# williamyang98/SDRPlusPlus-DAB-Radio-Plugin

Measured on AMD Instinct MI355X. Metric: DAB Mode-I frames/sec (OFDM+Viterbi), higher is better.
Workload: dtype f32

## Files before the change

sdrplusplus-dab-radio-plugin_amd/csrc/dabgpu_ctx.hpp:

```cpp
#pragma once
#include "../../include/dabgpu.h"

#include <hip/hip_runtime.h>

#include <chrono>
#include <map>
#include <memory>
#include <vector>

#include "dab_tables.hpp"
#include "kernels.hpp"
#include "iq_load.hpp"

namespace dabapi {

struct DeviceCode {
    dab::PunctureProfile prof;
    uint16_t *d_mother_pos = nullptr;
    uint8_t *d_prbs = nullptr;
    int32_t *d_punct_idx = nullptr;
    int32_t *d_fused_desc = nullptr, *d_fused_tiles = nullptr;
    dabk::LaneTables lane_tables() const { return dabk::LaneTables{d_punct_idx, d_fused_desc, d_fused_tiles}; }
    dabk::CodeTables tables(bool descramble) const {
        const bool chunked = d_mother_pos && prof.nsteps >= 102 && (prof.nsteps - 6) % 96 == 0;
// ... 41 lines not shown
    std::map<uint64_t, dabapi::DeviceCode *> code_by_descriptor;
    void *d_stage[9] = {nullptr, nullptr, nullptr, nullptr, nullptr, nullptr, nullptr, nullptr, nullptr};
    size_t stage_bytes[9] = {0, 0, 0, 0, 0, 0, 0, 0, 0};
    bool timing = false;
    dabapi::Timer timers[4];
    int ofdm_parts_override = 0;
    const unsigned long long *d_keep = nullptr;
    std::vector<void *> keep_tables;
    void *d_acq_scratch = nullptr;
    size_t acq_scratch_bytes = 0;
    void *d_lane_scratch = nullptr;
    size_t lane_scratch_bytes = 0;
    int lane_mode = -1;
    bool lane_unfused = false;
    bool test_one_domain = false;
    int test_fail_in = 0;
    int wave_slots = 3072;
    std::vector<dabgpu_bit_range> keep_ranges;
    dabk::StreamState *d_states = nullptr;
    int n_states = 0;
    hipEvent_t ev_states = nullptr;
    bool ev_states_pending = false;
    float thr_null_start = 0.35f;
    float signal_beta = 0.95f;
    bool loop_dd = false;
    float dd_gate = 2.5f;
    int keep_symbols = 75;
    struct SubHistory {
        int start_address, length;
        size_t bytes;
        int8_t *ring[2];
        int cur;
        bool live;
    };
    std::vector<SubHistory> sub_history;
    void *h_bounce = nullptr;
    size_t h_bounce_bytes = 0;
    unsigned long long signal_seq = 0;
    dabapi::Arena arena;
    dabapi::Pipeline *pipe = nullptr;
    int iq_format = 0;
};

namespace dabapi {

struct DeviceGuard {
    int prev = -1;
    bool switched = false;
    explicit DeviceGuard(const dabgpu_ctx *ctx) {
        if (ctx && hipGetDevice(&prev) == hipSuccess && prev != ctx->device) switched = hipSetDevice(ctx->device) == hipSuccess;
    }
    ~DeviceGuard() {
        if (switched) (void)hipSetDevice(prev);
    }
    DeviceGuard(const DeviceGuard &) = delete;
    DeviceGuard &operator=(const DeviceGuard &) = delete;
};

#define HIP_TRY(expr)                               \
    do {                                            \
        hipError_t e_ = (expr);                     \
        if (e_ != hipSuccess) return DABGPU_ERR_HIP; \
    } while (0)

struct ScopedTimer {
    dabgpu_ctx *ctx;
    int which;
    hipStream_t s;
    ScopedTimer(dabgpu_ctx *c, int w, hipStream_t st) : ctx(c), which(w), s(st) {
        if (ctx->timing) {
            Timer &t = ctx->timers[which];
            const int i = int(t.recorded % TIMER_RING);
            if (!t.start[i]) { (void)hipEventCreate(&t.start[i]); (void)hipEventCreate(&t.stop[i]); }
            t.has_mid[i] = false;
            (void)hipEventRecord(t.start[i], s);
        }
    }
    hipEvent_t *mids() {
        if (!ctx->timing) return nullptr;
        Timer &t = ctx->timers[which];
        const int i = int(t.recorded % TIMER_RING);
        for (hipEvent_t &e : t.mid[i])
            if (!e && hipEventCreate(&e) != hipSuccess) return nullptr;
        t.has_mid[i] = true;
        return t.mid[i];
    }
    ~ScopedTimer() {
        if (ctx->timing) {
            Timer &t = ctx->timers[which];
            (void)hipEventRecord(t.stop[int(t.recorded % TIMER_RING)], s);
            t.recorded++;
        }
    }
};

constexpr long SIGNAL_SPIN_US = 200;
inline int wait_for_signal(hipStream_t s, volatile unsigned long long *flag_host, unsigned long long *flag_dev, unsigned long long seq,
                           bool already_signalled = false, bool results_coherent = true) {
    if (!results_coherent) return hipStreamSynchronize(s) == hipSuccess ? DABGPU_OK : DABGPU_ERR_HIP;
    if (!already_signalled && dabk::launch_signal(flag_dev, seq, s) != hipSuccess) return DABGPU_ERR_HIP;
    const auto give_up = std::chrono::steady_clock::now() + std::chrono::microseconds(SIGNAL_SPIN_US);
    for (;;) {
        for (int i = 0; i < 64; i++) {
            if (*flag_host == seq) {
                __atomic_thread_fence(__ATOMIC_ACQUIRE);
                return DABGPU_OK;
            }
#if defined(__x86_64__) || defined(__i386__)
            __builtin_ia32_pause();
#endif
        }
        if (std::chrono::steady_clock::now() >= give_up) break;
    }
    return hipStreamSynchronize(s) == hipSuccess ? DABGPU_OK : DABGPU_ERR_HIP;
}

inline bool injected_failure(dabgpu_ctx *ctx) {
    return ctx->test_fail_in > 0 && --ctx->test_fail_in == 0;
}

inline hipStream_t pick_stream(dabgpu_ctx *ctx, void *stream) {
    return stream ? reinterpret_cast<hipStream_t>(stream) : ctx->stream;
}

int stage(dabgpu_ctx *ctx, int slot, size_t bytes, void **out);
int get_code(dabgpu_ctx *ctx, dab::PunctureProfile &&prof, DeviceCode **out);
void free_device_code(DeviceCode &dc);
void *device_alias_of_pinned(const void *host);
bool known_coherent_host(const void *host, size_t bytes);
int ensure_bounce(dabgpu_ctx *ctx, size_t bytes);
int note_state_use(dabgpu_ctx *ctx, hipStream_t s);
int wait_state_use(dabgpu_ctx *ctx);
void stats_of(const dabk::StreamState &st, dabgpu_stats *out);
void arena_destroy(dabgpu_ctx *ctx);
void pipeline_destroy(dabgpu_ctx *ctx);

inline bool subchannels_disjoint(const dabgpu_subchannel *sc, int n) {
    char used[864] = {};
    for (int i = 0; i < n; i++) {
        if (sc[i].start_address < 0 || sc[i].length <= 0 || sc[i].start_address + sc[i].length > 864) return false;
        for (int cu = sc[i].start_address; cu < sc[i].start_address + sc[i].length; cu++) {
            if (used[cu]) return false;
            used[cu] = 1;
        }
    }
    return true;
}

constexpr int LANE_MIN_CODEWORDS = 24576;

}
```

sdrplusplus-dab-radio-plugin_amd/csrc/dabgpu_decode_api.hip:

```cpp
#include "dabgpu_ctx.hpp"

#include <algorithm>
#include <cstring>

using namespace dab;
using namespace dabapi;

namespace {

bool use_lane(dabgpu_ctx *ctx, int nsteps, int n_codewords, hipStream_t s, dabk::LaneScratch *sc, int *rc, bool force = false) {
    *rc = DABGPU_OK;
    if (!dabk::lane_supported(nsteps)) return false;
    if (!force && (ctx->lane_mode == 0 || (ctx->lane_mode < 0 && n_codewords < LANE_MIN_CODEWORDS))) return false;
    const size_t need = dabk::lane_scratch_bytes(nsteps, n_codewords);
    if (ctx->lane_scratch_bytes < need) {
        if (hipStreamSynchronize(s) != hipSuccess) { *rc = DABGPU_ERR_HIP; return false; }
        if (ctx->d_lane_scratch) (void)hipFree(ctx->d_lane_scratch);
        ctx->d_lane_scratch = nullptr;
        ctx->lane_scratch_bytes = 0;
        if (hipMalloc(&ctx->d_lane_scratch, need) != hipSuccess) {
            ctx->d_lane_scratch = nullptr;
            if (ctx->lane_mode > 0 || force) *rc = DABGPU_ERR_NOMEM;
            return false;
        }
// ... 176 lines not shown
    if (nframes == 0) return DABGPU_OK;
    const size_t nb_soft = (nframes - 1) * soft_stride + NB_FRAME_BITS;
    const size_t nb_hist = size_t(n_streams) * 15 * sc->length * CU_BITS;
    const size_t nb_out = nframes * NB_CIFS * nbytes;
    void *d_soft, *d_hi = nullptr, *d_ho = nullptr, *d_out;
    int rc;
    if ((rc = stage(ctx, 1, nb_soft, &d_soft))) return rc;
    if ((rc = stage(ctx, 3, nb_out, &d_out))) return rc;
    if (history_in && (rc = stage(ctx, 4, nb_hist, &d_hi))) return rc;
    if (history_out && (rc = stage(ctx, 5, nb_hist, &d_ho))) return rc;
    hipStream_t s = ctx->stream;
    HIP_TRY(hipMemcpyAsync(d_soft, soft, nb_soft, hipMemcpyHostToDevice, s));
    if (history_in) HIP_TRY(hipMemcpyAsync(d_hi, history_in, nb_hist, hipMemcpyHostToDevice, s));
    rc = dabgpu_msc_decode_dev(ctx, sc, static_cast<const int8_t *>(d_soft), soft_stride, n_streams,
                               frames_per_stream, static_cast<const int8_t *>(d_hi), static_cast<int8_t *>(d_ho),
                               static_cast<uint8_t *>(d_out), s);
    if (rc) return rc;
    HIP_TRY(hipMemcpyAsync(out, d_out, nb_out, hipMemcpyDeviceToHost, s));
    if (history_out) HIP_TRY(hipMemcpyAsync(history_out, d_ho, nb_hist, hipMemcpyDeviceToHost, s));
    HIP_TRY(hipStreamSynchronize(s));
    return DABGPU_OK;
}

static int decode_grouped(dabgpu_ctx *ctx, uint8_t *d_fib, uint8_t *d_crc_ok, const dabgpu_subchannel *sc, int n_subchannels,
                          const int8_t *d_soft, size_t soft_stride, int n_streams, int frames_per_stream,
                          const int8_t *const *d_history_in, int8_t *const *d_history_out, uint8_t *const *d_out,
                          void *stream) {
    const int n_items = n_subchannels + (d_fib ? 1 : 0);
    if (n_items < 2 || ctx->lane_mode == 0 || ctx->lane_unfused || !d_soft || n_streams <= 0 || frames_per_stream <= 0 ||
        soft_stride < size_t(NB_FRAME_BITS))
        return 1;
    const long total_cw = long(n_items) * n_streams * frames_per_stream * NB_CIFS;
    if (ctx->lane_mode < 0 && total_cw < LANE_MIN_CODEWORDS) return 1;
    std::vector<dabk::LaneGroupItem> items;
    if (d_fib) {
        dabk::LaneGroupItem it{};
        it.code = ctx->fic.tables(true);
        it.tables = ctx->fic.lane_tables();
        it.args.soft = d_soft;
        it.args.soft_stride = soft_stride;
        it.args.n_streams = n_streams;
        it.args.frames_per_stream = frames_per_stream;
        it.args.out = d_fib;
        it.is_fic = true;
        it.crc_ok = d_crc_ok;
        if (((reinterpret_cast<uintptr_t>(d_soft) | soft_stride) & 15) || (reinterpret_cast<uintptr_t>(d_fib) & 3)) return 1;
        items.push_back(it);
    }
    for (int i = 0; i < n_subchannels; i++) {
        DeviceCode *dc = nullptr;
        const int rc = lookup_code(ctx, &sc[i], &dc);
        if (rc) return rc;
        dabk::LaneGroupItem it{};
        it.code = dc->tables(true);
        it.tables = dc->lane_tables();
        it.args.soft = d_soft;
        it.args.soft_stride = soft_stride;
        it.args.n_streams = n_streams;
        it.args.frames_per_stream = frames_per_stream;
        it.args.start_bit = sc[i].start_address * CU_BITS;
        it.args.nbits = sc[i].length * CU_BITS;
        it.args.hist_in = d_history_in ? d_history_in[i] : nullptr;
        it.args.hist_out = d_history_out ? d_history_out[i] : nullptr;
        it.args.out = d_out[i];
        if (it.args.hist_in && it.args.hist_in == it.args.hist_out) return DABGPU_ERR_ARG;
        if (!dabk::lane_supported(dc->prof.nsteps) || !dabk::lane_group_fusable(it.args)) return 1;
        items.push_back(it);
    }
    hipStream_t s = pick_stream(ctx, stream);
    const size_t need = dabk::lane_group_scratch_bytes(items.data(), n_items);
    if (ctx->lane_scratch_bytes < need) {
        HIP_TRY(hipStreamSynchronize(s));
        if (ctx->d_lane_scratch) (void)hipFree(ctx->d_lane_scratch);
        ctx->d_lane_scratch = nullptr;
        ctx->lane_scratch_bytes = 0;
        if (hipMalloc(&ctx->d_lane_scratch, need) != hipSuccess) {
            ctx->d_lane_scratch = nullptr;
            return 1;
        }
        ctx->lane_scratch_bytes = need;
    }
    ScopedTimer tm(ctx, 2, s);
    dabk::LaneScratch lsc{ctx->d_lane_scratch, ctx->lane_scratch_bytes};
    HIP_TRY(dabk::launch_lane_group(items.data(), n_items, lsc, s, tm.mids()));
    for (const dabk::LaneGroupItem &it : items)
        if (!it.is_fic) HIP_TRY(dabk::launch_msc_history(it.args, s));
    return 0;
}

static int decode_subchannels(dabgpu_ctx *ctx, const dabgpu_subchannel *sc, int n_subchannels, const int8_t *d_soft,
                              size_t soft_stride, int n_streams, int frames_per_stream, const int8_t *const *d_history_in,
                              int8_t *const *d_history_out, uint8_t *const *d_out, void *stream, uint8_t *d_fib = nullptr,
                              uint8_t *d_crc_ok = nullptr) {
    const long cw_each = long(n_streams) * frames_per_stream * NB_CIFS;
    bool group = n_subchannels >= 1 && n_subchannels + (d_fib ? 1 : 0) >= 2 && ctx->lane_mode <= 0 &&
                 (ctx->lane_mode == 0 || cw_each < LANE_MIN_CODEWORDS) && d_soft && n_streams > 0 && frames_per_stream > 0;
    std::vector<dabk::WaveGroupItem> items;
    for (int i = 0; group && i < n_subchannels; i++) {
        DeviceCode *dc = nullptr;
        const int rc = lookup_code(ctx, &sc[i], &dc);
        if (rc) return rc;
        if (!dabk::wave_group_supported(dc->prof.nsteps)) { group = false; break; }
        dabk::WaveGroupItem it{};
        it.code = dc->tables(true);
        it.args.soft = d_soft;
        it.args.soft_stride = soft_stride;
        it.args.n_streams = n_streams;
        it.args.frames_per_stream = frames_per_stream;
        it.args.start_bit = sc[i].start_address * CU_BITS;
        it.args.nbits = sc[i].length * CU_BITS;
        it.args.hist_in = d_history_in ? d_history_in[i] : nullptr;
        it.args.hist_out = d_history_out ? d_history_out[i] : nullptr;
        it.args.out = d_out[i];
        if (it.args.hist_in && it.args.hist_in == it.args.hist_out) return DABGPU_ERR_ARG;
        items.push_back(it);
    }
    if (group && n_subchannels == 1 && !dabk::wave_group_one_round(std::max(items[0].code.nsteps, ctx->fic.prof.nsteps), 2 * cw_each))
        group = false;
    if (group) {
        hipStream_t s = pick_stream(ctx, stream);
        ScopedTimer tm(ctx, 2, s);
        dabk::WaveFicItem fic{ctx->fic.tables(true), d_soft, soft_stride, n_streams * frames_per_stream, d_fib, d_crc_ok};
        HIP_TRY(dabk::launch_msc_decode_group(items.data(), int(items.size()), s, d_fib ? &fic : nullptr));
        return DABGPU_OK;
    }
    if (d_fib) {
        const int rc = dabgpu_fic_decode_dev(ctx, d_soft, soft_stride, n_streams * frames_per_stream, d_fib, d_crc_ok, stream);
        if (rc) return rc;
    }
    for (int i = 0; i < n_subchannels; i++) {
        const int rc = dabgpu_msc_decode_dev(ctx, &sc[i], d_soft, soft_stride, n_streams, frames_per_stream,
                                             d_history_in ? d_history_in[i] : nullptr,
                                             d_history_out ? d_history_out[i] : nullptr, d_out[i], stream);
        if (rc) return rc;
    }
    return DABGPU_OK;
}

int dabgpu_msc_decode_multi_dev(dabgpu_ctx *ctx, const dabgpu_subchannel *sc, int n_subchannels,
                                const int8_t *d_soft, size_t soft_stride, int n_streams, int frames_per_stream,
                                const int8_t *const *d_history_in, int8_t *const *d_history_out,
                                uint8_t *const *d_out, void *stream) {
    if (!ctx || !sc || !d_out || n_subchannels < 0) return DABGPU_ERR_ARG;
    DeviceGuard guard(ctx);
    std::vector<char> used(864, 0);
    for (int i = 0; i < n_subchannels; i++) {
        DeviceCode *dc = nullptr;
        const int rc = lookup_code(ctx, &sc[i], &dc);
        if (rc) return rc;
        if (!d_out[i]) return DABGPU_ERR_ARG;
        for (int cu = sc[i].start_address; cu < sc[i].start_address + sc[i].length; cu++) {
            if (used[cu]) return DABGPU_ERR_ARG;
            used[cu] = 1;
        }
    }
    {
        const int g = decode_grouped(ctx, nullptr, nullptr, sc, n_subchannels, d_soft, soft_stride, n_streams,
                                     frames_per_stream, d_history_in, d_history_out, d_out, stream);
        if (g <= 0) return g;
    }
    return decode_subchannels(ctx, sc, n_subchannels, d_soft, soft_stride, n_streams, frames_per_stream, d_history_in,
                              d_history_out, d_out, stream);
}

int dabgpu_decode_frames_dev(dabgpu_ctx *ctx, const int8_t *d_soft, size_t soft_stride, int n_streams,
                             int frames_per_stream, uint8_t *d_fib, uint8_t *d_crc_ok, const dabgpu_subchannel *sc,
                             int n_subchannels, const int8_t *const *d_history_in, int8_t *const *d_history_out,
// ... 452 lines not shown
```

sdrplusplus-dab-radio-plugin_amd/csrc/kernels.hpp:

```cpp
#pragma once
#include <hip/hip_runtime.h>

#include <vector>
#include <cstddef>
#include <cstdint>

namespace dabk {

struct OfdmTables {
    const float2 *twiddle;
    const uint16_t *bin_of_n;
    const uint16_t *n_of_vj;
};

struct StreamState {
    float fine_freq_offset;
    float coarse_freq_offset;
    float signal_average;
    float last_fine_error;
    int32_t total_frames_read;
    int32_t total_frames_desync;
    int32_t tracking;
    int32_t last_time_offset;
    double next_frame_start;
// ... 168 lines not shown
                              int max_out, int64_t advance, int only_lost, hipStream_t s);

struct SuperframeStatus {
    int32_t firecode_ok;
    int32_t rs_corrected;
    int32_t rs_uncorrectable;
    int32_t num_aus;
    int32_t au_crc_mask;
    int32_t au_start[8];
    int32_t reserved[3];
};
hipError_t launch_dabplus_superframes(const uint8_t *in, size_t in_stride, int n_superframes, int s, uint8_t *out,
                                      SuperframeStatus *status, hipStream_t stream, unsigned long long *done_flag = nullptr,
                                      unsigned long long done_seq = 0);

struct CodeTables {
    const uint16_t *mother_pos;
    int n_punct;
    int nsteps;
    const uint8_t *prbs_bytes;
    const uint16_t *chunk_first = nullptr;
};
__host__ __device__ inline int code_chunk_table_offset(int n_punct) { return (n_punct + 7) & ~7; }

hipError_t launch_fic_decode(const CodeTables &c, const int8_t *soft, size_t soft_stride, int n_frames,
                             uint8_t *fib, uint8_t *crc_ok, hipStream_t s);
hipError_t launch_viterbi_plain(const CodeTables &c, const int8_t *punct, int n_codewords, uint8_t *out,
                                hipStream_t s);
struct MscArgs {
    const int8_t *soft;
    size_t soft_stride;
    int n_streams;
    int frames_per_stream;
    int start_bit;
    int nbits;
    const int8_t *hist_in;
    int8_t *hist_out;
    uint8_t *out;
};
hipError_t launch_msc_decode(const CodeTables &c, const MscArgs &a, hipStream_t s);
struct WaveGroupItem {
    CodeTables code;
    MscArgs args;
};
struct WaveFicItem {
    CodeTables code;
    const int8_t *soft;
    size_t soft_stride;
    int n_frames;
    uint8_t *fib, *crc_ok;
};
bool wave_group_supported(int nsteps);
bool wave_group_one_round(int max_nsteps, long n_waves);
hipError_t launch_msc_decode_group(const WaveGroupItem *items, int n, hipStream_t s, const WaveFicItem *fic = nullptr);

struct LaneScratch {
    void *base;
    size_t bytes;
    bool unfused = false;
};
size_t lane_scratch_bytes(int nsteps, int n_codewords);
bool lane_supported(int nsteps);
struct LaneTables {
    const int32_t *punct_idx;
    const int32_t *fused_desc;
    const int32_t *fused_tiles;
};
void build_lane_fused_tables(const uint8_t *mask, int nsteps, std::vector<int32_t> &desc, std::vector<int32_t> &tiles);
hipError_t launch_fic_decode_lane(const CodeTables &c, const LaneTables &lt, const int8_t *soft, size_t soft_stride,
                                  int n_frames, const LaneScratch &sc, uint8_t *fib, uint8_t *crc_ok, hipStream_t s);
hipError_t launch_viterbi_plain_lane(const CodeTables &c, const LaneTables &lt, const int8_t *punct,
                                     int n_codewords, const LaneScratch &sc, uint8_t *out, hipStream_t s);
hipError_t launch_msc_decode_lane(const CodeTables &c, const LaneTables &lt, const MscArgs &a, const LaneScratch &sc,
                                  hipStream_t s);
struct LaneGroupItem {
    CodeTables code;
    LaneTables tables;
    MscArgs args;
    bool is_fic;
    uint8_t *crc_ok;
};
bool lane_group_fusable(const MscArgs &a);
size_t lane_group_scratch_bytes(const LaneGroupItem *items, int n);
hipError_t launch_lane_group(const LaneGroupItem *items, int n, const LaneScratch &sc, hipStream_t s, hipEvent_t *mid = nullptr);
size_t balanced_lds_bytes(unsigned grid, size_t lds, unsigned o_cap);
hipError_t launch_msc_history(const MscArgs &a, hipStream_t s);

struct MerSums {
    uint64_t signal, error;
    int32_t carriers, reserved;
};
hipError_t launch_mer(const int8_t *soft, size_t stride, int n_frames, int first_symbol, int n_symbols, MerSums *out,
                      hipStream_t s);
struct BerItem {
    int nsteps;
    const uint8_t *prbs_bytes;
    const int32_t *punct_idx;
    MscArgs args;
    bool is_fic;
    uint32_t *counts;
};
hipError_t launch_channel_ber(const BerItem *items, int n, hipStream_t s);
int ber_group_max();

constexpr int TII_COMBS = 24, TII_POSITIONS = 8, TII_CELLS = TII_COMBS * TII_POSITIONS, TII_PATTERNS = 70;
__host__ __device__ constexpr int tii_base(int q) { return q < 2 ? -768 + 384 * q : 384 * q - 767; }
__host__ __device__ constexpr int tii_pattern_mask(int p) {
    for (int v = 0, i = 0; v < 256; v++)
        if (__builtin_popcount(unsigned(v)) == 4 && i++ == p) return v;
    return -1;
}
constexpr int TII_WIN_BEGIN = 2352, TII_FLOOR_LO = 776, TII_FLOOR_HI = 927;
struct TiiRecord {
    float cell[TII_CELLS];
    float floor;
    int32_t frames;
    int32_t reserved[2];
};
struct TiiArgs {
    const float2 *iq;
    size_t stride;
    int n_streams, frames_per_stream;
    const float *freq_offset;
    const struct StreamState *state;
    const AcquiredFrame *acq;
    int timing_margin;
    TiiRecord *frame;
    TiiRecord *acc;
};
hipError_t launch_tii(const float2 *twiddle, const TiiArgs &a, hipStream_t s, int iq_format);

constexpr int CIR_WIN_BEGIN = 504, CIR_TAPS = 2048, CIR_CARRIERS = 1536;
struct CirRecord {
    float tap[CIR_TAPS];
    float carrier[CIR_CARRIERS];
    int32_t frames;
    int32_t reserved[3];
};
struct CirArgs {
    const float2 *iq;
    size_t stride;
    int n_streams, frames_per_stream;
    const float *freq_offset;
    const struct StreamState *state;
    const AcquiredFrame *acq;
    int timing_margin;
    const int8_t *prs_qt;
    CirRecord *frame;
    CirRecord *acc;
};
hipError_t launch_cir(const float2 *twiddle, const CirArgs &a, hipStream_t s, int iq_format);

hipError_t init_viterbi_kernel_attributes();
hipError_t init_lane_kernel_attributes();

inline size_t viterbi_wave_lds_bytes(int nsteps) { return size_t(nsteps) * 12 + 64; }
inline bool viterbi_fits(int nsteps) {
    const bool rot = nsteps >= 102 && (nsteps - 6) % 96 == 0;
    return 4 * size_t(nsteps) <= 65535 && (rot ? size_t(nsteps) * 8 + 4096 : viterbi_wave_lds_bytes(nsteps)) <= 160 * 1024;
}

}
```

sdrplusplus-dab-radio-plugin_amd/csrc/viterbi_lane_kernels.hip:

```cpp
#include <algorithm>
#include <type_traits>
#include <vector>

#include "mem_stream.hpp"
#include "kernels.hpp"
#include "dab_tables.hpp"
#include "soft_source.hpp"

namespace dabk {

using namespace dab;

namespace {

#ifndef LANE_FWD_ATTR
#define LANE_FWD_ATTR __attribute__((amdgpu_waves_per_eu(2, 2)))
#endif

constexpr int LANE_INIT2 = 2 * 6144;
constexpr int FT = 24;
constexpr int FCOLS = 8;
constexpr int FPITCH = FCOLS * 16 + 4;
constexpr int FERASED = FCOLS * 16;

// ... 302 lines not shown
    unsigned M[32];
#pragma unroll
    for (int r = 0; r < 32; r++) M[r] = pack16(-LANE_INIT2, -LANE_INIT2);
    M[0] = pack16(0, -LANE_INIT2);
    auto window_fence = [] {
        __builtin_amdgcn_fence(__ATOMIC_RELEASE, "wavefront");
        __builtin_amdgcn_fence(__ATOMIC_ACQUIRE, "wavefront");
    };
    fetch(0);
    stash();
    window_fence();
    const int dsh = desc_shift(src), dex = desc_extra(src);
    const int8_t *mys = reinterpret_cast<const int8_t *>(my);
    const int8_t *pcur[24];
    int32_t dnxt[24];
    auto soft_address = [&](int32_t d) {
        asm volatile("" : "+v"(d));
        return mys + (int((unsigned(d) >> dsh) & 0xFFFFu) + dex);
    };
#pragma unroll
    for (int j = 0; j < 24; j++) pcur[j] = soft_address(desc[j]);
    int tile = 0;
    for (int t0 = 0; t0 < nsteps; t0 += FT, tile++) {
        const bool more = t0 + FT < nsteps;
        if (more) fetch(tile + 1);
        const int t_end = min(t0 + FT, nsteps);
        for (int t = t0; t < t_end; t += 6) {
            const int32_t *dp = desc + 4 * min(t + 6, nsteps - 6);
#pragma unroll
            for (int j = 0; j < 24; j++) dnxt[j] = dp[j];
            __builtin_amdgcn_sched_barrier(0);
            Soft4 w[6];
#pragma unroll
            for (int i = 0; i < 6; i++) w[i] = Soft4{int(*pcur[4 * i]), int(*pcur[4 * i + 1]), int(*pcur[4 * i + 2]), int(*pcur[4 * i + 3])};
            lane_step<0>(M, w[0], dst + size_t(t + 0) * 64);
            lane_step<1>(M, w[1], dst + size_t(t + 1) * 64);
            lane_step<2>(M, w[2], dst + size_t(t + 2) * 64);
            lane_step<3>(M, w[3], dst + size_t(t + 3) * 64);
            lane_step<4>(M, w[4], dst + size_t(t + 4) * 64);
            lane_step<5>(M, w[5], dst + size_t(t + 5) * 64);
            if (((t / 6) & 1) == 1) {
                const unsigned ref = pack16(int(M[0]), int(M[0])) & 0xFFFEFFFEu;
#pragma unroll
                for (int r = 0; r < 32; r++) M[r] = pk_sub(M[r], ref);
            }
            __builtin_amdgcn_sched_barrier(0);
#pragma unroll
            for (int j = 0; j < 24; j++) pcur[j] = soft_address(dnxt[j]);
        }
        if (more) {
            window_fence();
            stash();
            window_fence();
        }
    }
}

template <class Src>
__global__ LANE_FWD_ATTR __launch_bounds__(256) void lane_forward_fused_kernel(Src src, const int32_t *desc, const int32_t *tiles,
                                                                 int nsteps, int groups, int n_codewords, uint2 *dec) {
    extern __shared__ __attribute__((aligned(16))) uint8_t fused_lds[];
    const int lane = threadIdx.x & 63;
    const int wv = threadIdx.x >> 6;
    const int group = __builtin_amdgcn_readfirstlane(blockIdx.x * 4 + wv);
    if (group >= groups) return;
    lane_forward_fused_body(src, desc, tiles, nsteps, group, n_codewords, dec, fused_lds + wv * ((64 + Src::PRE) * FPITCH),
                            lane);
}

constexpr int LANE_GROUP_MAX = 16;
struct LaneEntry {
    LSrcMsc src;
    const int32_t *desc, *tiles;
    const uint8_t *prbs;
    uint8_t *out;
    uint8_t *crc_ok;
    uint2 *dec;
    int nsteps, n_codewords, first_group, groups;
};
struct LaneEntryPack {
    int n;
    int total_groups;
    int prio_nsteps;
    LaneEntry e[LANE_GROUP_MAX];
};

__device__ __forceinline__ int find_entry(const LaneEntryPack &pack, int group) {
    int e = 0;
    while (e + 1 < pack.n && group >= pack.e[e + 1].first_group) e++;
    return e;
}

__global__ LANE_FWD_ATTR __launch_bounds__(256) void lane_forward_grouped_kernel(const LaneEntryPack pack) {
    extern __shared__ __attribute__((aligned(16))) uint8_t fused_lds[];
    const int lane = threadIdx.x & 63;
    const int wv = threadIdx.x >> 6;
    const int group = __builtin_amdgcn_readfirstlane(blockIdx.x * 4 + wv);
    if (group >= pack.total_groups) return;
    const LaneEntry &en = pack.e[find_entry(pack, group)];
    const LSrcMsc src = en.src;
    if (pack.prio_nsteps > 0 && en.nsteps >= pack.prio_nsteps) __builtin_amdgcn_s_setprio(1);
    lane_forward_fused_body(src, en.desc, en.tiles, en.nsteps, group - en.first_group, en.n_codewords, en.dec,
                            fused_lds + wv * ((64 + LSrcMsc::PRE) * FPITCH), lane);
}

__device__ __forceinline__ void lane_tb_step(const uint2 d, int t, int nsteps, unsigned &p, int &q, unsigned &word,
                                             uint32_t *row) {
    const unsigned rb = unsigned(q > 0 ? q - 1 : 0);
    const unsigned R = p >> 1;
    const unsigned I = ((R >> (rb + 1)) << rb) | (R & ((1u << rb) - 1u));
    const unsigned sel = (I & 8u) ? d.y : d.x;
    const unsigned h = (~sel >> (((((R >> rb) & 1u) << 1 | (p & 1u)) << 3) + (I & 7u))) & 1u;
    const unsigned b = (p >> q) & 1u;
    if (t < nsteps - 6) {
        word |= b << (31 - (t & 31));
        if ((t & 31) == 0) {
            row[t >> 5] = word;
            word = 0;
        }
    }
    p = (p & ~(1u << q)) | (h << q);
    q = (q == 5) ? 0 : q + 1;
}

template <int Q, int BIT>
__device__ __forceinline__ void lane_tb_step_static(const uint2 d, unsigned &p, unsigned &word) {
    constexpr unsigned rb = unsigned(Q > 0 ? Q - 1 : 0);
    const unsigned R = p >> 1;
    const unsigned I = ((R >> (rb + 1)) << rb) | (R & ((1u << rb) - 1u));
    const unsigned sel = (I & 8u) ? d.y : d.x;
    const unsigned h = (~sel >> (((((R >> rb) & 1u) << 1 | (p & 1u)) << 3) + (I & 7u))) & 1u;
    word |= ((p >> Q) & 1u) << BIT;
    p = (p & ~(1u << Q)) | (h << Q);
}

template <int Q0, int I>
__device__ __forceinline__ void lane_tb_block_steps(const uint2 (&d)[32], unsigned &p, unsigned &word) {
    if constexpr (I < 32) {
        lane_tb_step_static<(Q0 + I) % 6, I>(d[I], p, word);
        lane_tb_block_steps<Q0, I + 1>(d, p, word);
    }
}

__host__ __device__ __forceinline__ bool lane_tile_fits(int nsteps) {
    return size_t(64) * size_t(((nsteps - 6) >> 5) | 1) * 4 <= size_t(150) * 1024;
}

__device__ __forceinline__ unsigned crc16_byte_l(unsigned crc, unsigned byte) {
    crc = ((crc >> 8) | (crc << 8)) & 0xFFFFu;
    crc ^= byte;
    crc ^= (crc & 0xFFu) >> 4;
    crc ^= (crc << 12) & 0xFFFFu;
    crc ^= ((crc & 0xFFu) << 5) & 0xFFFFu;
    return crc;
}

__device__ __forceinline__ void lane_traceback_body(const uint2 *dec, int nsteps, int n_codewords, int group,
                                                    const uint8_t *prbs_bytes, uint8_t *out, uint8_t *crc_ok, uint32_t *tile,
                                                    int lane) {
    const uint2 *src = dec + size_t(group) * nsteps * 64 + lane;
    const int nwords = (nsteps - 6) >> 5;
    const int pitch = nwords | 1;
    const bool direct = tile == nullptr;
    const int nvalid_d = min(64, n_codewords - group * 64);
    const uint32_t *prbs32_d = reinterpret_cast<const uint32_t *>(prbs_bytes);
    uint32_t *out_d = reinterpret_cast<uint32_t *>(out + (size_t(group) * 64 + lane) * nwords * 4);
    uint32_t *row = direct ? nullptr : tile + lane * pitch;
    unsigned p = 0, word = 0;
    int q = 5 - ((nsteps - 1) % 6);
    uint2 d[32], dn[32];
#pragma unroll
    for (int i = 0; i < 6; i++) d[i] = ld_stream(src + size_t(nsteps - 1 - i) * 64);
#pragma unroll
    for (int i = 0; i < 32; i++) dn[i] = ld_stream(src + size_t(nsteps - 7 - i) * 64);
#pragma unroll
    for (int i = 0; i < 6; i++) lane_tb_step(d[i], nsteps - 1 - i, nsteps, p, q, word, row);
    auto block = [&](auto q0, int t1) {
#pragma unroll
        for (int i = 0; i < 32; i++) d[i] = dn[i];
        if (t1 >= 32) {
#pragma unroll
            for (int i = 0; i < 32; i++) dn[i] = ld_stream(src + size_t(t1 - 32 - i) * 64);
        }
        unsigned w = 0;
        lane_tb_block_steps<decltype(q0)::value, 0>(d, p, w);
        if (!direct) {
            row[t1 >> 5] = w;
        } else if (lane < nvalid_d) {
            uint32_t v = __builtin_bswap32(w);
            if (prbs32_d) v ^= prbs32_d[t1 >> 5];
            out_d[t1 >> 5] = v;
        }
    };
    for (int t1 = nsteps - 7; t1 >= 0; t1 -= 96) {
        block(std::integral_constant<int, 0>{}, t1);
        block(std::integral_constant<int, 2>{}, t1 - 32);
        block(std::integral_constant<int, 4>{}, t1 - 64);
    }
    if (direct) return;
    __syncthreads();
    const int nvalid = min(64, n_codewords - group * 64);
    const uint32_t *prbs32 = reinterpret_cast<const uint32_t *>(prbs_bytes);
    uint32_t *out32 = reinterpret_cast<uint32_t *>(out + size_t(group) * 64 * nwords * 4);
    for (int i = lane; i < nvalid * nwords; i += 64) {
        const int r = i / nwords, w = i - r * nwords;
        uint32_t v = __builtin_bswap32(tile[r * pitch + w]);
        if (prbs32) v ^= prbs32[w];
        out32[i] = v;
        if (crc_ok) tile[r * pitch + w] = v;
    }
    if (crc_ok) {
        __syncthreads();
        const int nfib = nwords >> 3;
        for (int j = lane; j < nvalid * nfib; j += 64) {
            const int r = j / nfib, fi = j - r * nfib;
            const uint32_t *wp = tile + r * pitch + 8 * fi;
            unsigned crc = 0xFFFFu;
#pragma unroll
            for (int k = 0; k < 30; k++) crc = crc16_byte_l(crc, (wp[k >> 2] >> (8 * (k & 3))) & 0xFFu);
            const unsigned rx = ((wp[7] >> 16) & 0xFFu) << 8 | (wp[7] >> 24);
            crc_ok[(size_t(group) * 64) * nfib + j] = uint8_t((crc ^ 0xFFFFu) == rx);
        }
    }
}

__global__ __launch_bounds__(64) void lane_traceback_kernel(const uint2 *dec, int nsteps, int n_codewords,
                                                            const uint8_t *prbs_bytes, uint8_t *out, uint8_t *crc_ok) {
    extern __shared__ uint32_t tile[];
    lane_traceback_body(dec, nsteps, n_codewords, blockIdx.x, prbs_bytes, out, crc_ok, lane_tile_fits(nsteps) ? tile : nullptr,
                        threadIdx.x);
}

__global__ __launch_bounds__(64) void lane_traceback_grouped_kernel(const LaneEntryPack pack) {
    extern __shared__ uint32_t tile[];
    const int group = blockIdx.x;
    const LaneEntry &en = pack.e[find_entry(pack, group)];
    lane_traceback_body(en.dec, en.nsteps, en.n_codewords, group - en.first_group, en.prbs, en.out, en.crc_ok,
                        lane_tile_fits(en.nsteps) ? tile : nullptr, threadIdx.x);
}

template <class Src>
hipError_t run_lane(Src f, bool vec16, bool fusable, const CodeTables &c, const LaneTables &lt, int n_codewords,
                    const LaneScratch &sc, uint8_t *out, uint8_t *crc_ok, hipStream_t s) {
    const int groups = (n_codewords + 63) / 64;
    const int nwords = (c.nsteps - 6) >> 5;
    const size_t need = lane_scratch_bytes(c.nsteps, n_codewords);
    if (!sc.base || sc.bytes < need || (reinterpret_cast<uintptr_t>(out) & 3)) return hipErrorInvalidValue;
    uint32_t *M = reinterpret_cast<uint32_t *>(sc.base);
    uint2 *dec = reinterpret_cast<uint2 *>(M + size_t(groups) * c.nsteps * 64);
    const unsigned fgrid = unsigned((groups + 3) / 4);
    if (fusable && vec16 && lt.fused_desc && lt.fused_tiles && !sc.unfused) {
        const size_t lds = balanced_lds_bytes(fgrid, size_t(4) * (64 + Src::PRE) * FPITCH, 3);
        hipLaunchKernelGGL((lane_forward_fused_kernel<Src>), dim3(fgrid), dim3(256), lds, s, f, lt.fused_desc, lt.fused_tiles,
                           c.nsteps, groups, n_codewords, dec);
    } else {
        hipLaunchKernelGGL((lane_prep_kernel<Src>), dim3(unsigned((c.nsteps + PREP_STEPS - 1) / PREP_STEPS), unsigned(groups)),
                           dim3(256), 0, s, f, lt.punct_idx, c.nsteps, n_codewords, int(vec16), M);
        const size_t fwd_lds = balanced_lds_bytes(fgrid, 0, 8);
        hipLaunchKernelGGL(lane_forward_kernel, dim3(fgrid), dim3(256), fwd_lds, s, M, c.nsteps, groups, dec);
    }
    const size_t tb_lds = lane_tile_fits(c.nsteps) ? size_t(64) * (nwords | 1) * 4 : 0;
    hipLaunchKernelGGL(lane_traceback_kernel, dim3(unsigned(groups)), dim3(64), tb_lds, s, dec, c.nsteps, n_codewords,
                       c.prbs_bytes, out, crc_ok);
    return hipGetLastError();
}

inline bool aligned16(const void *p, size_t stride) { return ((reinterpret_cast<uintptr_t>(p) | stride) & 15) == 0; }

}

hipError_t init_lane_kernel_attributes() {
    for (const void *k : {reinterpret_cast<const void *>(lane_forward_kernel),
                          reinterpret_cast<const void *>(lane_forward_fused_kernel<LSrcFic>),
                          reinterpret_cast<const void *>(lane_forward_fused_kernel<LSrcPlain>),
                          reinterpret_cast<const void *>(lane_forward_fused_kernel<LSrcMsc>),
                          reinterpret_cast<const void *>(lane_forward_grouped_kernel),
                          reinterpret_cast<const void *>(lane_traceback_kernel),
                          reinterpret_cast<const void *>(lane_traceback_grouped_kernel)}) {
        const hipError_t e = hipFuncSetAttribute(k, hipFuncAttributeMaxDynamicSharedMemorySize, 160 * 1024);
        if (e != hipSuccess) return e;
    }
    return hipSuccess;
}

size_t lane_scratch_bytes(int nsteps, int n_codewords) {
    const size_t groups = size_t((n_codewords + 63) / 64);
    const size_t nwords = size_t((nsteps - 6) >> 5);
    (void)nwords;
    return groups * 64 * size_t(nsteps) * 12 + 256;
}

bool lane_supported(int nsteps) {
    return nsteps >= 38 && nsteps % 6 == 0 && ((nsteps - 6) & 31) == 0;
}

hipError_t launch_fic_decode_lane(const CodeTables &c, const LaneTables &lt, const int8_t *soft, size_t soft_stride,
                                  int n_frames, const LaneScratch &sc, uint8_t *fib, uint8_t *crc_ok, hipStream_t s) {
    return run_lane(LSrcFic{soft, soft_stride}, aligned16(soft, soft_stride), true, c, lt, n_frames * NB_FIC_GROUPS, sc,
                    fib, crc_ok, s);
}

hipError_t launch_viterbi_plain_lane(const CodeTables &c, const LaneTables &lt, const int8_t *punct,
                                     int n_codewords, const LaneScratch &sc, uint8_t *out, hipStream_t s) {
    return run_lane(LSrcPlain{punct, c.n_punct}, aligned16(punct, size_t(c.n_punct)), true, c, lt, n_codewords, sc, out,
                    nullptr, s);
}

hipError_t launch_msc_decode_lane(const CodeTables &c, const LaneTables &lt, const MscArgs &a, const LaneScratch &sc,
                                  hipStream_t s) {
    const LSrcMsc f = make_msc_src(a);
    const bool fusable = (a.frames_per_stream * NB_CIFS) % 64 == 0 &&
                         (!a.hist_in || ((reinterpret_cast<uintptr_t>(a.hist_in) | size_t(a.nbits)) & 15) == 0);
    return run_lane(f, aligned16(a.soft, a.soft_stride) && (a.start_bit & 15) == 0, fusable, c, lt,
                    a.n_streams * a.frames_per_stream * NB_CIFS, sc, a.out, nullptr, s);
}

bool lane_group_fusable(const MscArgs &a) {
    return (a.frames_per_stream * NB_CIFS) % 64 == 0 && aligned16(a.soft, a.soft_stride) && (a.start_bit & 15) == 0 &&
           (!a.hist_in || ((reinterpret_cast<uintptr_t>(a.hist_in) | size_t(a.nbits)) & 15) == 0) &&
           (reinterpret_cast<uintptr_t>(a.out) & 3) == 0;
}

static size_t item_codewords(const LaneGroupItem &it) {
    return size_t(it.args.n_streams) * it.args.frames_per_stream * NB_CIFS;
}

size_t lane_group_scratch_bytes(const LaneGroupItem *items, int n) {
    size_t total = 0;
    for (int i = 0; i < n; i++) total += ((item_codewords(items[i]) + 63) / 64) * 64 * size_t(items[i].code.nsteps) * sizeof(uint2);
    return total + 512;
}

static int resident_cus() {
    static const int n = [] {
        int dev = 0;
        hipDeviceProp_t prop;
        return (hipGetDevice(&dev) == hipSuccess && hipGetDeviceProperties(&prop, dev) == hipSuccess && prop.multiProcessorCount > 0)
                   ? prop.multiProcessorCount : 256;
    }();
    return n;
}

hipError_t launch_lane_group(const LaneGroupItem *items, int n, const LaneScratch &sc, hipStream_t s, hipEvent_t *mid) {
    if (n <= 0) return hipSuccess;
    if (!sc.base || sc.bytes < lane_group_scratch_bytes(items, n)) return hipErrorInvalidValue;
    char *p = static_cast<char *>(sc.base);
    for (int i0 = 0; i0 < n; i0 += LANE_GROUP_MAX) {
        LaneEntryPack pack{};
        pack.n = std::min(LANE_GROUP_MAX, n - i0);
        int max_nwords = 0;
        for (int i = 0; i < pack.n; i++) {
            const LaneGroupItem &it = items[i0 + i];
            const MscArgs &a = it.args;
            if (!it.tables.fused_desc || !it.tables.fused_tiles || !lane_supported(it.code.nsteps)) return hipErrorInvalidValue;
            LaneEntry &e = pack.e[i];
            e.n_codewords = int(item_codewords(it));
            if (it.is_fic) {
                if (!aligned16(a.soft, a.soft_stride) || (reinterpret_cast<uintptr_t>(a.out) & 3)) return hipErrorInvalidValue;
                e.src = make_fic_src(a.soft, a.soft_stride, e.n_codewords);
            } else {
                if (!lane_group_fusable(a)) return hipErrorInvalidValue;
                e.src = make_msc_src(a);
            }
            e.desc = it.tables.fused_desc;
            e.tiles = it.tables.fused_tiles;
            e.prbs = it.code.prbs_bytes;
            e.out = a.out;
            e.crc_ok = it.is_fic ? it.crc_ok : nullptr;
            e.dec = reinterpret_cast<uint2 *>(p);
            e.nsteps = it.code.nsteps;
            e.first_group = pack.total_groups;
            e.groups = (e.n_codewords + 63) / 64;
            pack.total_groups += e.groups;
            p += size_t(e.groups) * 64 * size_t(e.nsteps) * sizeof(uint2);
            if (lane_tile_fits(e.nsteps)) max_nwords = std::max(max_nwords, (e.nsteps - 6) >> 5);
        }
        const unsigned fgrid = unsigned((pack.total_groups + 3) / 4);
        const size_t lds = balanced_lds_bytes(fgrid, size_t(4) * (64 + LSrcMsc::PRE) * FPITCH, 3);
        {
            int longest = 0, shortest = 0x7fffffff;
            for (int i = 0; i < pack.n; i++) { longest = std::max(longest, pack.e[i].nsteps); shortest = std::min(shortest, pack.e[i].nsteps); }
            pack.prio_nsteps = (pack.total_groups <= 2 * 4 * resident_cus() && longest > shortest) ? longest : 0;
        }
        const bool timed = mid && i0 + LANE_GROUP_MAX >= n;
        hipLaunchKernelGGL(lane_forward_grouped_kernel, dim3(fgrid), dim3(256), lds, s, pack);
        if (timed) (void)hipEventRecord(mid[0], s);
        const size_t tb_lds = size_t(64) * (max_nwords | 1) * 4;
        hipLaunchKernelGGL(lane_traceback_grouped_kernel, dim3(unsigned(pack.total_groups)), dim3(64), tb_lds, s, pack);
        if (timed) (void)hipEventRecord(mid[1], s);
    }
    return hipGetLastError();
}

void build_lane_fused_tables(const uint8_t *mask, int nsteps, std::vector<int32_t> &desc, std::vector<int32_t> &tiles) {
    std::vector<int> idx(size_t(4) * nsteps, -1);
    for (int p = 0, j = 0; p < 4 * nsteps; p++)
        if (mask[p]) idx[p] = j++;
    const int ntiles = (nsteps + FT - 1) / FT;
    desc.assign(size_t(4) * nsteps, FERASED | (FERASED << 16));
    tiles.assign(size_t(2) * ntiles, 0);
    for (int tile = 0; tile < ntiles; tile++) {
        const int p0 = 4 * FT * tile, p1 = std::min(4 * nsteps, p0 + 4 * FT);
        int lo = -1, hi = 0;
        for (int p = p0; p < p1; p++)
            if (idx[p] >= 0) { if (lo < 0) lo = idx[p]; hi = idx[p] + 1; }
        if (lo < 0) continue;
        const int lo_al = lo & ~15;
        tiles[2 * tile] = lo_al;
        tiles[2 * tile + 1] = (hi - lo_al + 15) / 16;
        for (int p = p0; p < p1; p++) {
            if (idx[p] < 0) continue;
            const int d = tdi_delay(idx[p]);
            const int col = idx[p] - lo_al;
            desc[p] = (int(d) * FPITCH + col) | (col << 16);
        }
    }
}

}
```

Measured before the change: 2.455 million.

## Fuse traceback into forward kernel for long-code priority waves

When a group mixes code lengths and total work is small, waves running the longest (priority) codes now run their Viterbi traceback inside the forward kernel, using a wave-scope fence instead of a block barrier. Entries are reordered so untraced groups come first, and the separate traceback kernel is launched only over those. This targets the tail latency of the longest codewords, which otherwise wait for a second launch. In exchange, per-wave LDS grows to fit the traceback tile, which may reduce occupancy, and the timing-event bookkeeping becomes more complex.

```diff
diff --git a/sdrplusplus-dab-radio-plugin_amd/csrc/dabgpu_ctx.hpp b/sdrplusplus-dab-radio-plugin_amd/csrc/dabgpu_ctx.hpp
--- a/sdrplusplus-dab-radio-plugin_amd/csrc/dabgpu_ctx.hpp
+++ b/sdrplusplus-dab-radio-plugin_amd/csrc/dabgpu_ctx.hpp
@@ -147,8 +147,10 @@
         const int i = int(t.recorded % TIMER_RING);
         for (hipEvent_t &e : t.mid[i])
             if (!e && hipEventCreate(&e) != hipSuccess) return nullptr;
-        t.has_mid[i] = true;
         return t.mid[i];
+    }
+    void mids_recorded(bool both) {
+        if (ctx->timing) ctx->timers[which].has_mid[int(ctx->timers[which].recorded % TIMER_RING)] = both;
     }
     ~ScopedTimer() {
         if (ctx->timing) {
diff --git a/sdrplusplus-dab-radio-plugin_amd/csrc/dabgpu_decode_api.hip b/sdrplusplus-dab-radio-plugin_amd/csrc/dabgpu_decode_api.hip
--- a/sdrplusplus-dab-radio-plugin_amd/csrc/dabgpu_decode_api.hip
+++ b/sdrplusplus-dab-radio-plugin_amd/csrc/dabgpu_decode_api.hip
@@ -282,7 +282,9 @@
     }
     ScopedTimer tm(ctx, 2, s);
     dabk::LaneScratch lsc{ctx->d_lane_scratch, ctx->lane_scratch_bytes};
-    HIP_TRY(dabk::launch_lane_group(items.data(), n_items, lsc, s, tm.mids()));
+    bool split = false;
+    HIP_TRY(dabk::launch_lane_group(items.data(), n_items, lsc, s, tm.mids(), &split));
+    tm.mids_recorded(split);
     for (const dabk::LaneGroupItem &it : items)
         if (!it.is_fic) HIP_TRY(dabk::launch_msc_history(it.args, s));
     return 0;
diff --git a/sdrplusplus-dab-radio-plugin_amd/csrc/kernels.hpp b/sdrplusplus-dab-radio-plugin_amd/csrc/kernels.hpp
--- a/sdrplusplus-dab-radio-plugin_amd/csrc/kernels.hpp
+++ b/sdrplusplus-dab-radio-plugin_amd/csrc/kernels.hpp
@@ -274,7 +274,8 @@
 };
 bool lane_group_fusable(const MscArgs &a);
 size_t lane_group_scratch_bytes(const LaneGroupItem *items, int n);
-hipError_t launch_lane_group(const LaneGroupItem *items, int n, const LaneScratch &sc, hipStream_t s, hipEvent_t *mid = nullptr);
+hipError_t launch_lane_group(const LaneGroupItem *items, int n, const LaneScratch &sc, hipStream_t s, hipEvent_t *mid = nullptr,
+                             bool *mid_recorded = nullptr);
 size_t balanced_lds_bytes(unsigned grid, size_t lds, unsigned o_cap);
 hipError_t launch_msc_history(const MscArgs &a, hipStream_t s);
 
diff --git a/sdrplusplus-dab-radio-plugin_amd/csrc/viterbi_lane_kernels.hip b/sdrplusplus-dab-radio-plugin_amd/csrc/viterbi_lane_kernels.hip
--- a/sdrplusplus-dab-radio-plugin_amd/csrc/viterbi_lane_kernels.hip
+++ b/sdrplusplus-dab-radio-plugin_amd/csrc/viterbi_lane_kernels.hip
@@ -408,6 +408,8 @@
     int n;
     int total_groups;
     int prio_nsteps;
+    int wave_lds;
+    int tb_tile;
     LaneEntry e[LANE_GROUP_MAX];
 };
 
@@ -415,19 +417,6 @@
     int e = 0;
     while (e + 1 < pack.n && group >= pack.e[e + 1].first_group) e++;
     return e;
-}
-
-__global__ LANE_FWD_ATTR __launch_bounds__(256) void lane_forward_grouped_kernel(const LaneEntryPack pack) {
-    extern __shared__ __attribute__((aligned(16))) uint8_t fused_lds[];
-    const int lane = threadIdx.x & 63;
-    const int wv = threadIdx.x >> 6;
-    const int group = __builtin_amdgcn_readfirstlane(blockIdx.x * 4 + wv);
-    if (group >= pack.total_groups) return;
-    const LaneEntry &en = pack.e[find_entry(pack, group)];
-    const LSrcMsc src = en.src;
-    if (pack.prio_nsteps > 0 && en.nsteps >= pack.prio_nsteps) __builtin_amdgcn_s_setprio(1);
-    lane_forward_fused_body(src, en.desc, en.tiles, en.nsteps, group - en.first_group, en.n_codewords, en.dec,
-                            fused_lds + wv * ((64 + LSrcMsc::PRE) * FPITCH), lane);
 }
 
 __device__ __forceinline__ void lane_tb_step(const uint2 d, int t, int nsteps, unsigned &p, int &q, unsigned &word,
@@ -481,6 +470,12 @@
     return crc;
 }
 
+__device__ __forceinline__ void lane_wave_fence() {
+    __builtin_amdgcn_fence(__ATOMIC_RELEASE, "wavefront");
+    __builtin_amdgcn_fence(__ATOMIC_ACQUIRE, "wavefront");
+}
+
+template <bool WAVE>
 __device__ __forceinline__ void lane_traceback_body(const uint2 *dec, int nsteps, int n_codewords, int group,
                                                     const uint8_t *prbs_bytes, uint8_t *out, uint8_t *crc_ok, uint32_t *tile,
                                                     int lane) {
@@ -524,7 +519,8 @@
         block(std::integral_constant<int, 4>{}, t1 - 64);
     }
     if (direct) return;
-    __syncthreads();
+    auto barrier = [] { if constexpr (WAVE) lane_wave_fence(); else __syncthreads(); };
+    barrier();
     const int nvalid = min(64, n_codewords - group * 64);
     const uint32_t *prbs32 = reinterpret_cast<const uint32_t *>(prbs_bytes);
     uint32_t *out32 = reinterpret_cast<uint32_t *>(out + size_t(group) * 64 * nwords * 4);
@@ -536,7 +532,7 @@
         if (crc_ok) tile[r * pitch + w] = v;
     }
     if (crc_ok) {
-        __syncthreads();
+        barrier();
         const int nfib = nwords >> 3;
         for (int j = lane; j < nvalid * nfib; j += 64) {
             const int r = j / nfib, fi = j - r * nfib;
@@ -553,16 +549,36 @@
 __global__ __launch_bounds__(64) void lane_traceback_kernel(const uint2 *dec, int nsteps, int n_codewords,
                                                             const uint8_t *prbs_bytes, uint8_t *out, uint8_t *crc_ok) {
     extern __shared__ uint32_t tile[];
-    lane_traceback_body(dec, nsteps, n_codewords, blockIdx.x, prbs_bytes, out, crc_ok, lane_tile_fits(nsteps) ? tile : nullptr,
-                        threadIdx.x);
+    lane_traceback_body<false>(dec, nsteps, n_codewords, blockIdx.x, prbs_bytes, out, crc_ok,
+                               lane_tile_fits(nsteps) ? tile : nullptr, threadIdx.x);
+}
+
+__global__ LANE_FWD_ATTR __launch_bounds__(256) void lane_forward_grouped_kernel(const LaneEntryPack pack) {
+    extern __shared__ __attribute__((aligned(16))) uint8_t fused_lds[];
+    const int lane = threadIdx.x & 63;
+    const int wv = threadIdx.x >> 6;
+    const int group = __builtin_amdgcn_readfirstlane(blockIdx.x * 4 + wv);
+    if (group >= pack.total_groups) return;
+    const LaneEntry &en = pack.e[find_entry(pack, group)];
+    const LSrcMsc src = en.src;
+    const bool prio = pack.prio_nsteps > 0 && en.nsteps >= pack.prio_nsteps;
+    if (prio) __builtin_amdgcn_s_setprio(1);
+    uint8_t *win = fused_lds + wv * pack.wave_lds;
+    lane_forward_fused_body(src, en.desc, en.tiles, en.nsteps, group - en.first_group, en.n_codewords, en.dec, win, lane);
+    if (!prio) return;
+    __builtin_amdgcn_s_setprio(0);
+    asm volatile("s_waitcnt vmcnt(0)" ::: "memory");
+    lane_wave_fence();
+    lane_traceback_body<true>(en.dec, en.nsteps, en.n_codewords, group - en.first_group, en.prbs, en.out, en.crc_ok,
+                              pack.tb_tile ? reinterpret_cast<uint32_t *>(win) : nullptr, lane);
 }
 
 __global__ __launch_bounds__(64) void lane_traceback_grouped_kernel(const LaneEntryPack pack) {
     extern __shared__ uint32_t tile[];
     const int group = blockIdx.x;
     const LaneEntry &en = pack.e[find_entry(pack, group)];
-    lane_traceback_body(en.dec, en.nsteps, en.n_codewords, group - en.first_group, en.prbs, en.out, en.crc_ok,
-                        lane_tile_fits(en.nsteps) ? tile : nullptr, threadIdx.x);
+    lane_traceback_body<false>(en.dec, en.nsteps, en.n_codewords, group - en.first_group, en.prbs, en.out, en.crc_ok,
+                               lane_tile_fits(en.nsteps) ? tile : nullptr, threadIdx.x);
 }
 
 template <class Src>
@@ -667,19 +683,26 @@
     return n;
 }
 
-hipError_t launch_lane_group(const LaneGroupItem *items, int n, const LaneScratch &sc, hipStream_t s, hipEvent_t *mid) {
+hipError_t launch_lane_group(const LaneGroupItem *items, int n, const LaneScratch &sc, hipStream_t s, hipEvent_t *mid,
+                             bool *mid_recorded) {
+    if (mid_recorded) *mid_recorded = false;
     if (n <= 0) return hipSuccess;
     if (!sc.base || sc.bytes < lane_group_scratch_bytes(items, n)) return hipErrorInvalidValue;
+    if (n > LANE_GROUP_MAX) mid = nullptr;
+    bool recorded = mid != nullptr;
     char *p = static_cast<char *>(sc.base);
+    constexpr int WINDOW = (64 + LSrcMsc::PRE) * FPITCH;
     for (int i0 = 0; i0 < n; i0 += LANE_GROUP_MAX) {
         LaneEntryPack pack{};
         pack.n = std::min(LANE_GROUP_MAX, n - i0);
-        int max_nwords = 0;
+        LaneEntry ent[LANE_GROUP_MAX];
+        int total_groups = 0, longest = 0, shortest = 0x7fffffff;
         for (int i = 0; i < pack.n; i++) {
             const LaneGroupItem &it = items[i0 + i];
             const MscArgs &a = it.args;
             if (!it.tables.fused_desc || !it.tables.fused_tiles || !lane_supported(it.code.nsteps)) return hipErrorInvalidValue;
-            LaneEntry &e = pack.e[i];
+            LaneEntry &e = ent[i];
+            e = LaneEntry{};
             e.n_codewords = int(item_codewords(it));
             if (it.is_fic) {
                 if (!aligned16(a.soft, a.soft_stride) || (reinterpret_cast<uintptr_t>(a.out) & 3)) return hipErrorInvalidValue;
@@ -695,26 +718,44 @@
             e.crc_ok = it.is_fic ? it.crc_ok : nullptr;
             e.dec = reinterpret_cast<uint2 *>(p);
             e.nsteps = it.code.nsteps;
-            e.first_group = pack.total_groups;
             e.groups = (e.n_codewords + 63) / 64;
-            pack.total_groups += e.groups;
+            total_groups += e.groups;
             p += size_t(e.groups) * 64 * size_t(e.nsteps) * sizeof(uint2);
-            if (lane_tile_fits(e.nsteps)) max_nwords = std::max(max_nwords, (e.nsteps - 6) >> 5);
+            longest = std::max(longest, e.nsteps);
+            shortest = std::min(shortest, e.nsteps);
+        }
+        pack.prio_nsteps = (total_groups <= 2 * 4 * resident_cus() && longest > shortest) ? longest : 0;
+        int untraced_groups = 0, max_nwords = 0, k = 0;
+        for (int pass = 0; pass < 2; pass++)
+            for (int i = 0; i < pack.n; i++) {
+                const bool traced = pack.prio_nsteps > 0 && ent[i].nsteps >= pack.prio_nsteps;
+                if (traced != (pass == 1)) continue;
+                LaneEntry &e = pack.e[k++];
+                e = ent[i];
+                e.first_group = pack.total_groups;
+                pack.total_groups += e.groups;
+                if (!traced) {
+                    untraced_groups += e.groups;
+                    if (lane_tile_fits(e.nsteps)) max_nwords = std::max(max_nwords, (e.nsteps - 6) >> 5);
+                }
+            }
+        pack.wave_lds = WINDOW;
+        if (pack.prio_nsteps > 0) {
+            const int tile = 64 * (((longest - 6) >> 5) | 1) * 4;
+            pack.tb_tile = 4 * std::max(WINDOW, tile) <= 160 * 1024 / 2;
+            if (pack.tb_tile) pack.wave_lds = (std::max(WINDOW, tile) + 15) & ~15;
         }
         const unsigned fgrid = unsigned((pack.total_groups + 3) / 4);
-        const size_t lds = balanced_lds_bytes(fgrid, size_t(4) * (64 + LSrcMsc::PRE) * FPITCH, 3);
-        {
-            int longest = 0, shortest = 0x7fffffff;
-            for (int i = 0; i < pack.n; i++) { longest = std::max(longest, pack.e[i].nsteps); shortest = std::min(shortest, pack.e[i].nsteps); }
-            pack.prio_nsteps = (pack.total_groups <= 2 * 4 * resident_cus() && longest > shortest) ? longest : 0;
-        }
-        const bool timed = mid && i0 + LANE_GROUP_MAX >= n;
+        const size_t lds = balanced_lds_bytes(fgrid, size_t(4) * pack.wave_lds, 3);
         hipLaunchKernelGGL(lane_forward_grouped_kernel, dim3(fgrid), dim3(256), lds, s, pack);
-        if (timed) (void)hipEventRecord(mid[0], s);
-        const size_t tb_lds = size_t(64) * (max_nwords | 1) * 4;
-        hipLaunchKernelGGL(lane_traceback_grouped_kernel, dim3(unsigned(pack.total_groups)), dim3(64), tb_lds, s, pack);
-        if (timed) (void)hipEventRecord(mid[1], s);
-    }
+        if (mid) recorded = hipEventRecord(mid[0], s) == hipSuccess;
+        if (untraced_groups > 0) {
+            const size_t tb_lds = size_t(64) * (max_nwords | 1) * 4;
+            hipLaunchKernelGGL(lane_traceback_grouped_kernel, dim3(unsigned(untraced_groups)), dim3(64), tb_lds, s, pack);
+        }
+        if (mid) recorded = hipEventRecord(mid[1], s) == hipSuccess && recorded;
+    }
+    if (mid_recorded) *mid_recorded = recorded;
     return hipGetLastError();
 }
 
```

After: 2.486 million (median of 6 runs). +1.2%, better.
